# Gteam1-EE/srsRAN_Project_23.5

Hardware: AMD Instinct MI355X
Metric: LDPC info-bits/sec + OFDM slots/sec, 100 MHz n78 273-PRB grid (higher is better)
Workload: dtype int8; 1 GPU; 273-PRB 30kHz PUSCH, 256QAM R=948/1024, 1 layer, 38 CB/slot BG1 Z=384, TBS 319784; per slot, time-domain samples to transport block: OFDM demod (4096-pt, 1 port) + DM-RS channel estimate + equalise/soft-demap/descramble + rate-dematch + LDPC decode (6 it, early_stop=0) + TB assembly/CRC24A; slots synthesised by the transmit chain + AWGN; parallelism=slots sharded across GPUs, no data-path collective

## Files before the change

srsran_project_23.5_amd/csrc/ldpc_decode_pk.hip:

```cpp
#include "miphy_internal.h"
#include "rdm_device.h"
#include "ldpc_frame_device.h"
#include <algorithm>
#include <cstdlib>

namespace {

__device__ __forceinline__ bool block_crc_is_zero(const int8_t* soft, const miphy_graph_tables* __restrict__ tab, int zi, int order, int L,
                                                  uint32_t* red, int tid, int nt)
{
  return block_xor(crc_zmask_partial(soft, tab, zi, order, L, tid, nt), red, tid, nt) == 0;
}

__device__ __forceinline__ uint32_t block_crc(const int8_t* soft, const miphy_graph_tables* __restrict__ tab, int crc_id, uint32_t poly,
                                              uint32_t order, int K, int L, uint32_t* red, int tid, int nt)
{
  return block_xor(crc_div_partial(soft, tab, crc_id, poly, order, K, L, tid, nt), red, tid, nt);
}

#ifdef LDPC_PK_PROFILE
__device__ unsigned long long g_ldpc_prof[2048 * 8];
#define PROF_T(var) const unsigned long long var = __builtin_amdgcn_s_memtime()
#define PROF_ADD(slot, a, b) prof_acc[slot] += (unsigned long long)((b) - (a))
#define PROF_COUNT()                                              \
  do {                                                            \
    if (tid == 0 && blockIdx.x < 2048) {                          \
      for (int q = 0; q < 7; ++q)                                 \
        g_ldpc_prof[blockIdx.x * 8 + q] += prof_acc[q];           \
      g_ldpc_prof[blockIdx.x * 8 + 7] += 1;                       \
    }                                                             \
    for (int q = 0; q < 7; ++q)                                   \
      prof_acc[q] = 0;                                            \
  } while (0)
#else
#define PROF_T(var)
#define PROF_ADD(slot, a, b)
#define PROF_COUNT()
#endif

#define LDPC_PK_MIN_WAVES_PLAIN 4
#ifndef LDPC_PK_MIN_WAVES_SPLIT
#define LDPC_PK_MIN_WAVES_SPLIT 3
#endif
#ifndef LDPC_PK_MIN_WAVES_FUSED
#define LDPC_PK_MIN_WAVES_FUSED 3
#endif
struct raw_in16 {
  uint32_t a0, a1, a2, a3, e;
};
__device__ __forceinline__ raw_in16 load_in16_raw(const int8_t* __restrict__ in, int mb, int v)
{
  const uint32_t* p4 = reinterpret_cast<const uint32_t*>(in - mb) + 4 * v;
  const rdm_u4    a  = *reinterpret_cast<const rdm_u4*>(p4);
  raw_in16        r;
  r.a0 = a.x, r.a1 = a.y, r.a2 = a.z, r.a3 = a.w;
  r.e  = (mb != 0) ? p4[4] : 0u;
  return r;
}
__device__ __forceinline__ uint4 shift_in16(const raw_in16& r, int mb)
{
  if (mb == 0)
    return make_uint4(r.a0, r.a1, r.a2, r.a3);
  return make_uint4(__builtin_amdgcn_alignbyte(r.a1, r.a0, mb), __builtin_amdgcn_alignbyte(r.a2, r.a1, mb), __builtin_amdgcn_alignbyte(r.a3, r.a2, mb),
                    __builtin_amdgcn_alignbyte(r.e, r.a3, mb));
}
constexpr int PK_PRE = 3;

__device__ __forceinline__ int pk_in16_vectors(int mb, int E)
{
  return (mb == 0) ? (E >> 4) : ((E >= 4) ? ((E - 4) >> 4) : 0);
}
__device__ __forceinline__ void pk_prefetch(raw_in16 (&pre)[PK_PRE], uint32_t c, uint32_t n, const miphy_ldpc_rdm_desc* __restrict__ rdm,
                                            const int8_t* __restrict__ rm_in_base, const uint32_t* __restrict__ cb_order, int tid, int nt)
{
#pragma unroll
  for (int k = 0; k < PK_PRE; ++k)
    pre[k] = raw_in16{0, 0, 0, 0, 0};
  if (c < n) {
    const miphy_ldpc_rdm_desc r  = load_words(rdm + (cb_order ? cb_order[c] : c));
    const int8_t*             in = rm_in_base + r.in_offset;
    const int                 mb = (int)(((uintptr_t)in) & 3), nq = pk_in16_vectors(mb, (int)r.E);
#pragma unroll
    for (int k = 0; k < PK_PRE; ++k) {
      pre[k] = raw_in16{0, 0, 0, 0, 0};
      if (tid + k * nt < nq)
        pre[k] = load_in16_raw(in, mb, tid + k * nt);
    }
  }
}

typedef __attribute__((address_space(1))) const int8_t* global_ci8;
__device__ __attribute__((noinline)) void pk_fused_load(int8_t* __restrict__ soft, global_ci8 in_global, int E, int F, int mod, int Z, int bgK, int soft_bytes,
                                                        raw_in16 p0, raw_in16 p1, raw_in16 p2, int tid, int nt)
{
  static_assert(PK_PRE == 3, "three prefetched vectors are passed by value");
  const int8_t* __restrict__ in = (const int8_t*)in_global;
    int stid = tid;
    asm volatile("" : "+v"(stid));
    const int                 mb  = (int)(((uintptr_t)in) & 3);
    const int                 nq  = pk_in16_vectors(mb, E);
    int8_t*                   img = soft + 2 * Z;
    rm_geom                   g;
    g.r0 = 0, g.f1 = (bgK - 2) * Z, g.f0 = g.f1 - F, g.F = F, g.E = E, g.mod = mod, g.Kq = E / mod;
    image_access ia;
    ia.jbase = 0;
    {
      uint4* z4 = reinterpret_cast<uint4*>(soft);
      for (int k = stid; k < (2 * Z) >> 4; k += nt)
        z4[k] = make_uint4(0, 0, 0, 0);
      for (int k = g.f0 + stid; k < g.f1; k += nt)
        img[k] = 127;
      for (int k = 2 * Z + E + F + stid; k < soft_bytes; k += nt)
        soft[k] = 0;
    }
    switch (mod) {
#define PK_STAGE(MOD)                                                                         \
  case MOD:                                                                                   \
    _Pragma("unroll") for (int k = 0; k < PK_PRE; ++k) if (stid + k * nt < nq)                 \
        stage_vector<MOD>(ia, img, g, F, stid + k * nt, shift_in16(k == 0 ? p0 : (k == 1 ? p1 : p2), mb));               \
    for (int v = stid + PK_PRE * nt; v < nq; v += nt)                                          \
      stage_vector<MOD>(ia, img, g, F, v, load_in16(in, mb, v));                              \
    break;
      PK_STAGE(8)
      PK_STAGE(6)
      PK_STAGE(4)
      PK_STAGE(2)
      default:
        PK_STAGE(1)
#undef PK_STAGE
    }
    for (int k = (nq << 4) + stid; k < E; k += nt) {
      const int p = k / (int)mod, q = k - p * (int)mod;
      const int r = q * g.Kq + p;
      img[r + ((r >= g.f0) ? F : 0)] = in[k];
    }
    __syncthreads();
}

__device__ __forceinline__ int pk_fused_image_out(const int8_t* __restrict__ soft, int8_t* __restrict__ llr_img, int Z, int bgi, int in_len, int tid, int nt)
{
  typedef uint32_t u32x4 __attribute__((ext_vector_type(4)));
  int          last = 0;
  u32x4*       dst  = reinterpret_cast<u32x4*>(llr_img);
  const uint4* src  = reinterpret_cast<const uint4*>(soft + 2 * Z);
  const int    nimg = in_len >> 4, nall = ((miphy_bg_N_short(bgi) * Z) >> 4);
  asm volatile("" : "+v"(tid));
  for (int q = tid; q < nimg; q += nt) {
    const uint4 v = src[q];
    const u32x4 o = {v.x, v.y, v.z, v.w};
    __builtin_nontemporal_store(o, dst + q);
    last = last_nonzero_behind(v, q, last);
  }
  const u32x4 zero = {0, 0, 0, 0};
  for (int q = nimg + tid; q < nall; q += nt)
    __builtin_nontemporal_store(zero, dst + q);
  return last;
}

constexpr int PK_ATAB_DEGREE = MIPHY_LDPC_ADR_TABLE_DEGREE, PK_ATAB_QUADS = (PK_ATAB_DEGREE + 3) / 4;
template <bool FUSED, bool GMSG, int PARTS = 1, bool ATAB = false, bool RSKIP = false>
__global__ void __launch_bounds__(192 * PARTS, PARTS > 1 ? LDPC_PK_MIN_WAVES_SPLIT : (FUSED ? LDPC_PK_MIN_WAVES_FUSED : LDPC_PK_MIN_WAVES_PLAIN))
ldpc_decode_pk_kernel(const miphy_ldpc_dec_desc* __restrict__ descs,
                      const miphy_graph_tables* __restrict__ tab,
                      const int8_t* __restrict__ llr_base,
                      uint8_t* __restrict__ out_base,
                      int32_t* __restrict__ iters_out,
                      int max_nodes,
                      const uint32_t* __restrict__ harq_slot,
                      uint8_t* __restrict__ harq_crc_ok,
                      uint32_t n,
                      uint32_t* __restrict__ queue,
                      const miphy_ldpc_rdm_desc* __restrict__ rdm,
                      const int8_t* __restrict__ rm_in_base,
                      uint32_t* __restrict__ gmsg,
                      int gmsg_pairs,
                      int lds_pairs,
                      const uint32_t* __restrict__ cb_order,
                      const pk_adr_quad* const* __restrict__ adr_by_z)
{
  extern __shared__ __attribute__((aligned(16))) unsigned char smem[];
  const int tid = threadIdx.x;
  const int nt  = blockDim.x;
  constexpr bool SPLIT = PARTS > 1;
  static_assert(PARTS == 1 || PARTS == 2 || PARTS == 4, "parts of the latency form");
  static_assert(!(SPLIT && GMSG), "the latency form keeps its messages in LDS");
  static_assert(!ATAB || (FUSED && !GMSG && !SPLIT), "address tables: the throughput form that dematches, messages in LDS");
  static_assert(!(RSKIP && (SPLIT || GMSG)), "visits are left out by the throughput forms with their messages in LDS");
  const int nth  = nt / PARTS;
  const int part = SPLIT ? __builtin_amdgcn_readfirstlane((tid >= nth) + (PARTS > 2 ? (tid >= 2 * nth) + (tid >= 3 * nth) : 0)) : 0;
  const int lr   = tid - part * nth;
  raw_in16  pre[PK_PRE];
  if (FUSED)
    pk_prefetch(pre, blockIdx.x, n, rdm, rm_in_base, cb_order, tid, nt);
#ifdef LDPC_PK_PROFILE
  unsigned long long prof_acc[7] = {};
#endif
  for (uint32_t q = blockIdx.x; q < n;) {
  __builtin_amdgcn_s_setprio(LDPC_PK_SETPRIO_OUT);
  PROF_T(p_start);
  const uint32_t cb = cb_order ? cb_order[q] : q;
  const miphy_ldpc_dec_desc dsc = load_words(descs + cb);
  const int                 Z   = dsc.Z;
  const int                 H   = (Z + 1) >> 1;
  const int                 bgi = (dsc.bg == 1) ? 0 : 1;
  const int                 bgK = miphy_bg_K(bgi);
  const int                 bgM = miphy_bg_M(bgi);
  const int                 K   = bgK * Z;
  const int                 zp  = tab->z_pos[Z];

  int8_t*   soft       = reinterpret_cast<int8_t*>(smem);
  const int lay_alloc  = miphy_ldpc_layers(bgi, max_nodes);
  const int soft_bytes = miphy_ldpc_soft_bytes(bgi, lay_alloc, Z);
  const int pairs_all  = tab->pair_start[bgi][lay_alloc];
  const int pairs_lds  = GMSG ? lds_pairs : pairs_all;
  uint32_t* c2v_lane   = reinterpret_cast<uint32_t*>(smem + soft_bytes) + (lr >> 6) * (pairs_lds * 64) + (lr & 63);
  uint32_t* c2v_glob   = GMSG ? gmsg + ((size_t)blockIdx.x * (nt >> 6) + (tid >> 6)) * ((size_t)gmsg_pairs * 64) + (tid & 63) - 64 * (size_t)pairs_lds : nullptr;
  uint32_t* red        = reinterpret_cast<uint32_t*>(smem + soft_bytes) + (nth >> 6) * (pairs_lds * 64);
  uint32_t* xch = red + 16 + lr;

  __syncthreads();
  if (tid == 0) {
    const uint32_t ticket = atomicAdd(queue, 1u);
    if (ticket == n - 1u)
      *queue = 0u;
    red[15] = gridDim.x + ticket;
  }
  if (!FUSED && harq_crc_ok && harq_crc_ok[harq_slot[cb]]) {
    if (tid == 0)
      iters_out[cb] = -1;
    __syncthreads();
    q = red[15];
    continue;
  }
  const int8_t* llr    = llr_base + dsc.llr_offset;
  uint8_t*      out    = out_base + dsc.out_offset;
  const int     in_len = (int)dsc.in_len;

  if (tid < 15)
    red[tid] = 0;
  int last = 0;
  auto prefetch = [&](uint32_t c) { pk_prefetch(pre, c, n, rdm, rm_in_base, cb_order, tid, nt); };
  pk_adr_quad    anx[ATAB ? PK_ATAB_QUADS : 1];
  pk_adr_row     atab    = pk_adr_row();
  const uint32_t astride = 16u * (uint32_t)nt, alayer = PK_ATAB_QUADS * astride;
  if (ATAB) {
    const int zq = __builtin_amdgcn_readfirstlane(Z >> 4), bytes = __builtin_amdgcn_readfirstlane(lay_alloc * (int)alayer);
    atab.rsrc    = __builtin_amdgcn_make_buffer_rsrc(const_cast<pk_adr_quad*>(adr_by_z[zq]), 0, bytes, 0x00020000);
    atab.soff = alayer;
    pk_table_request<PK_ATAB_DEGREE>(anx, atab, 16u * (uint32_t)tid, astride);
  }
  if (FUSED) {
    const miphy_ldpc_rdm_desc rd = load_words(rdm + cb);
    pk_fused_load(soft, (global_ci8)(rm_in_base + rd.in_offset), (int)rd.E, (int)dsc.nof_filler_bits, (int)rd.mod, Z, bgK, soft_bytes, pre[0], pre[1], pre[2], tid, nt);
    last = pk_fused_image_out(soft, const_cast<int8_t*>(llr), Z, bgi, in_len, tid, nt);
  } else {
    last = cb_plain_load(soft, llr, in_len, Z, soft_bytes, tid, nt);
  }
  atomicMax(reinterpret_cast<int*>(&red[0]), last);
  __syncthreads();
  last = (int)red[0];

  const bool use_crc = dsc.crc_poly != MIPHY_CRC_NONE;
  if (last == 0) {
    if (!use_crc) {
      store_all_ones(out, K, tid, nt);
    }
    if (tid == 0) {
      iters_out[cb] = 0;
      if (FUSED && harq_crc_ok)
        harq_crc_ok[harq_slot[cb]] = 0;
    }
    if (FUSED)
      prefetch(red[15]);
    q = red[15];
    continue;
  }
  const int nof_layers = cb_nof_layers(last, Z, bgi);

  const uint32_t* edges_g   = tab->edge_sb[bgi][zp];
  uint32_t lay_info = 0;
  {
    const int ml = tid & 63;
    if (ml < bgM) {
      const uint32_t e0 = tab->row_start[bgi][ml];
      lay_info          = e0 | (((uint32_t)tab->row_start[bgi][ml + 1] - e0) << 10) | ((uint32_t)tab->pair_start[bgi][ml] << 16);
    }
  }
  uint32_t        poly = 0, order = 0;
  int             L = 0;
  if (use_crc) {
    poly  = tab->crc_poly[dsc.crc_poly];
    order = tab->crc_order[dsc.crc_poly];
    L     = K - dsc.nof_filler_bits;
  }
  const bool final_only = use_crc && (dsc.flags & 1u);
  const int zi = (use_crc && L <= 32 * MIPHY_CRC_ZMASK_WORDS) ? miphy_crc_zmask_index(dsc.crc_poly) : -1;

  int       result_iters = 0;
  const int max_iter     = dsc.max_iter;
  PROF_T(p_loaded);
  PROF_ADD(0, p_start, p_loaded);
  int Zv = Z, Hv = (lr + H < Z) ? H : 0;
#ifndef LDPC_PK_SCALAR_WRAP
  asm volatile("" : "+v"(Zv), "+v"(Hv));
#endif
  __builtin_amdgcn_s_setprio(LDPC_PK_SETPRIO1);
  part_edges<PARTS> pe;
  if (SPLIT)
    load_part_edges<PARTS>(pe, edges_g, (uint32_t)__builtin_amdgcn_readlane((int)lay_info, 1), part);
  [[maybe_unused]] uint64_t sat_layers = 0;
  for (int it = 0; it < max_iter; ++it) {
    for (int m = (it == 0) ? 1 : 0; m < nof_layers; ++m) {
      const uint32_t  li    = (uint32_t)__builtin_amdgcn_readlane((int)lay_info, m);
      const int       e0    = (int)(li & 0x3ffu);
      const int       d     = (int)((li >> 10) & 0x3fu);
      const uint32_t* edges = edges_g + 2 * e0;
      PROF_T(p_l0);
      if constexpr (SPLIT) {
        part_edges<PARTS> pn;
        const uint32_t    lin  = (uint32_t)__builtin_amdgcn_readlane((int)lay_info, (m + 1 < nof_layers) ? m + 1 : 0);
        auto              next = [&]() { load_part_edges<PARTS>(pn, edges_g, lin, part); };
        const pk_exchange<decltype(next)> x = {xch, part, nth, lr < H, next};
        uint32_t* cl = c2v_lane + 64 * (li >> 16);
        if (it == 0 || (it == 1 && m == 0))
          update_rows_pk_split<true, PARTS>(pe, soft, cl, lr, Hv, Zv, x);
        else
          update_rows_pk_split<false, PARTS>(pe, soft, cl, lr, Hv, Zv, x);
        pe = pn;
      } else if constexpr (!RSKIP) {
        if (ATAB) {
          if (tid < H)
            update_rows_pk_visit_tab<PK_ATAB_DEGREE>(it, m, soft, c2v_lane + 64 * (li >> 16),
                                                     pk_adr_table{anx, {atab.rsrc, (uint32_t)__builtin_amdgcn_readfirstlane((m + 1 < nof_layers) ? m + 1 : 0) * alayer},
                                                                  16u * (uint32_t)tid, astride});
        } else if (tid < H) {
          if (GMSG && (int)(li >> 16) >= pairs_lds) {
            update_rows_pk_visit<FUSED>(it, m, d, soft, c2v_glob + 64 * (li >> 16), pk_adr_computed{edges, tid, Hv, Zv, 0});
          } else {
            update_rows_pk_visit<FUSED>(it, m, d, soft, c2v_lane + 64 * (li >> 16), pk_adr_computed{edges, tid, Hv, Zv, 0});
          }
        }
      } else if (!((sat_layers >> m) & 1u)) {
        bool all_inf = false;
        if (ATAB) {
          const uint64_t live = ~sat_layers & (((uint64_t)1 << nof_layers) - 1u), above = live & ~(((uint64_t)2 << m) - 1u);
          const int      mn   = __builtin_amdgcn_readfirstlane(above ? __builtin_ctzll(above) : __builtin_ctzll(live));
          if (tid < H)
            all_inf = update_rows_pk_visit_tab<PK_ATAB_DEGREE, true>(it, m, soft, c2v_lane + 64 * (li >> 16),
                                                                     pk_adr_table{anx, {atab.rsrc, (uint32_t)mn * alayer}, 16u * (uint32_t)tid, astride});
        } else if (tid < H) {
          if (GMSG && (int)(li >> 16) >= pairs_lds) {
            all_inf = update_rows_pk_visit<FUSED, true>(it, m, d, soft, c2v_glob + 64 * (li >> 16), pk_adr_computed{edges, tid, Hv, Zv, 0});
          } else {
            all_inf = update_rows_pk_visit<FUSED, true>(it, m, d, soft, c2v_lane + 64 * (li >> 16), pk_adr_computed{edges, tid, Hv, Zv, 0});
          }
        }
        if (__builtin_amdgcn_ballot_w64(tid < H && !all_inf) == 0)
          sat_layers |= (uint64_t)1 << m;
      }
      PROF_T(p_l1);
      __syncthreads();
      PROF_T(p_l2);
      PROF_ADD(1, p_l0, p_l1);
      PROF_ADD(2, p_l1, p_l2);
    }
    if (use_crc && !final_only) {
      if (zi >= 0 ? block_crc_is_zero(soft, tab, zi, (int)order, L, red, tid, nt) : block_crc(soft, tab, dsc.crc_poly, poly, order, K, L, red, tid, nt) == 0) {
        result_iters = it + 1;
        break;
      }
    }
  }
  PROF_T(p_dec);
  __builtin_amdgcn_s_setprio(LDPC_PK_SETPRIO_OUT);
  if (FUSED) {
    prefetch(red[15]);
  }
  if (final_only)
    result_iters = (zi >= 0 ? block_crc_is_zero(soft, tab, zi, (int)order, L, red, tid, nt) : block_crc(soft, tab, dsc.crc_poly, poly, order, K, L, red, tid, nt) == 0)
                       ? max_iter
                       : 0;
  PROF_T(p_crc);
  PROF_ADD(3, p_dec, p_crc);

  store_hard_words(soft, out, K, tid, nt);
  if (tid == 0) {
    iters_out[cb] = result_iters;
    if (harq_crc_ok && (FUSED || result_iters > 0))
      harq_crc_ok[harq_slot[cb]] = result_iters > 0;
  }
  PROF_T(p_end);
  PROF_ADD(4, p_crc, p_end);
  PROF_ADD(5, p_start, p_end);
  PROF_COUNT();
  q = red[15];
  }
}

struct pk_instance_key {
  bool fused, gmsg;
  int  parts;
  bool atab, row_skip;
  constexpr bool operator==(const pk_instance_key& o) const { return fused == o.fused && gmsg == o.gmsg && parts == o.parts && atab == o.atab && row_skip == o.row_skip; }
};
typedef decltype(&ldpc_decode_pk_kernel<false, false>) pk_kernel_fn;
struct pk_instance {
  pk_instance_key key;
  pk_kernel_fn    kernel;
};
template <bool FUSED, bool GMSG, int PARTS = 1, bool ATAB = false, bool RSKIP = false>
constexpr pk_instance pk_instance_of()
{
  return {{FUSED, GMSG, PARTS, ATAB, RSKIP}, ldpc_decode_pk_kernel<FUSED, GMSG, PARTS, ATAB, RSKIP>};
}
constexpr pk_instance pk_instances[] = {
    pk_instance_of<false, false>(),        pk_instance_of<false, true>(),         pk_instance_of<true, false>(),         pk_instance_of<true, true>(),
    pk_instance_of<false, false, 2>(),     pk_instance_of<true, false, 2>(),      pk_instance_of<false, false, 4>(),     pk_instance_of<true, false, 4>(),
    pk_instance_of<true, false, 1, true>(), pk_instance_of<false, false, 1, false, true>(), pk_instance_of<true, false, 1, false, true>(),
    pk_instance_of<true, false, 1, true, true>(),
};

}

#ifdef LDPC_PK_PROFILE
extern "C" int miphy_debug_ldpc_profile(unsigned long long out[8], int reset)
{
  static unsigned long long h[2048 * 8];
  if (hipMemcpyFromSymbol(h, HIP_SYMBOL(g_ldpc_prof), sizeof(h)) != hipSuccess)
    return -1;
  for (int q = 0; q < 8; ++q) {
    out[q] = 0;
    for (int b = 0; b < 2048; ++b)
      out[q] += h[b * 8 + q];
  }
  if (reset) {
    for (auto& v : h)
      v = 0;
    if (hipMemcpyToSymbol(HIP_SYMBOL(g_ldpc_prof), h, sizeof(h)) != hipSuccess)
      return -1;
  }
  return 0;
}
#endif

#ifdef LDPC_PK_PROFILE2
extern "C" int miphy_debug_ldpc_profile2(unsigned long long out[8], int reset)
{
  if (hipMemcpyFromSymbol(out, HIP_SYMBOL(g_ldpc_prof2), 8 * sizeof(unsigned long long)) != hipSuccess)
    return -1;
  if (reset) {
    unsigned long long z[8] = {};
    if (hipMemcpyToSymbol(HIP_SYMBOL(g_ldpc_prof2), z, sizeof(z)) != hipSuccess)
      return -1;
  }
  return 0;
}
#endif

int miphy_ldpc_pk_waves_per_cu(bool fused, int parts)
{
#ifdef LDPC_PK_REPORT_WAVES_FUSED
  if (fused && parts <= 1)
    return 4 * LDPC_PK_REPORT_WAVES_FUSED;
#endif
  return 4 * (parts > 1 ? LDPC_PK_MIN_WAVES_SPLIT : (fused ? LDPC_PK_MIN_WAVES_FUSED : LDPC_PK_MIN_WAVES_PLAIN));
}

size_t miphy_ldpc_pk_lds_bytes(int bgi, int lay, size_t Zt, int pairs_all, int parts)
{
  const size_t waves = ((Zt + 1) / 2 + 63) / 64;
  return (size_t)miphy_ldpc_soft_bytes(bgi, lay, (int)Zt) + waves * (size_t)pairs_all * 256 + 64 + (parts > 1 ? (size_t)parts * 3 * 64 * waves * 4 : 0);
}

int miphy_ldpc_pk_per_cu(size_t lds, int waves, bool fused, int parts)
{
  return std::max(1, std::min((int)((size_t)160 * 1024 / lds), miphy_ldpc_pk_waves_per_cu(fused, parts) / waves));
}

uint32_t miphy_ldpc_pk_grid(const miphy_ctx* ctx, uint32_t n, int threads, size_t lds, bool fused, int parts)
{
  return std::min<uint32_t>(n, (uint32_t)(ctx->num_cus * miphy_ldpc_pk_per_cu(lds, threads / 64, fused, parts)));
}

int miphy_ldpc_pk_launch(miphy_ctx* ctx, const miphy_ldpc_launch& L, const miphy_ldpc_dec_desc* d_descs, const uint32_t* d_order, const int8_t* llr,
                         uint8_t* out_bits, int32_t* iters, const uint32_t* harq_slot, uint8_t* harq_crc_ok, const miphy_ldpc_rdm_desc* d_rdm,
                         const int8_t* rm_in, void* gmsg, hipStream_t s)
{
  const bool fused = (L.used & MIPHY_LDPC_KERNEL_FUSED) != 0, gm = L.gmsg_pairs > 0;
  MIPHY_REQUIRE(L.threads <= 1024, "ldpc_decode: workgroup of %d threads", L.threads);
  const pk_instance_key want = {fused, gm, L.parts, L.adr_by_z != nullptr, L.row_skip};
  pk_kernel_fn          kern = nullptr;
  for (const pk_instance& i : pk_instances)
    if (i.key == want)
      kern = i.kernel;
  MIPHY_REQUIRE(kern, "ldpc_decode: no packed kernel instance {fused %d, global messages %d, parts %d, address table %d, row skip %d}", want.fused, want.gmsg, want.parts,
                want.atab, want.row_skip);
  if (L.lds > 48 * 1024) {
    MIPHY_HIP_CHECK(hipFuncSetAttribute((const void*)kern, hipFuncAttributeMaxDynamicSharedMemorySize, (int)L.lds));
  }
  uint32_t* queue = nullptr;
  int       rc    = miphy_next_queue_counter(ctx, &queue);
  if (rc)
    return rc;
  hipLaunchKernelGGL(kern, dim3(L.grid), dim3(L.threads), L.lds, s, d_descs, ctx->d_tables, llr, out_bits, iters, L.nodes, harq_slot, harq_crc_ok, L.c.count, queue, d_rdm,
                     rm_in, (uint32_t*)gmsg, L.gmsg_pairs, gm ? L.lds_pairs : 0, d_order, (const pk_adr_quad* const*)L.adr_by_z);
  MIPHY_HIP_CHECK(hipGetLastError());
  return MIPHY_OK;
}
```

srsran_project_23.5_amd/csrc/ldpc_pk_device.h:

```cpp
#pragma once
#include "miphy_internal.h"
#include <type_traits>

namespace {

typedef short s16x2 __attribute__((ext_vector_type(2)));

__device__ __forceinline__ s16x2 as_s2(uint32_t x)
{
  return __builtin_bit_cast(s16x2, x);
}
__device__ __forceinline__ uint32_t as_u(s16x2 x)
{
  return __builtin_bit_cast(uint32_t, x);
}
__device__ __forceinline__ s16x2 splat(int c)
{
  return s16x2{(short)c, (short)c};
}
__device__ __forceinline__ s16x2 pk_min(s16x2 a, s16x2 b)
{
  return __builtin_elementwise_min(a, b);
}
__device__ __forceinline__ s16x2 pk_max(s16x2 a, s16x2 b)
// ... 324 lines not shown
    }
  }
  __builtin_amdgcn_s_setprio(LDPC_PK_SETPRIO2);
  if constexpr (ATAB)
    pk_table_request<D>(adr.q, adr.next, adr.voff, adr.stride);
  const uint32_t sA = ((uint32_t)(uint16_t)mag.x * 52428u) >> 16, sB = ((uint32_t)(uint16_t)mag.y * 52428u) >> 16;
  const s16x2    pm = pk_ashr15(as_s2(spx));
  const s16x2    c  = as_s2((sA | (sB << 16)) ^ as_u(pm)) - pm;
  const uint32_t r  = as_u(c);
  c2v[0] = ZE ? c2v_pack(splat(0), c) : c2v_pack(c, splat(0));
#pragma unroll
  for (int jj = 1; jj < (D + 1) / 2; ++jj)
    c2v[64 * jj] = 0u;
  pk_soft_bit<ATAB>(soft, adrA[ZE]) = (int8_t)r;
  pk_soft_bit<ATAB>(soft, adrB[ZE]) = (int8_t)(r >> 16);
  __builtin_amdgcn_s_setprio(LDPC_PK_SETPRIO1);
}

template <typename MID>
__device__ __forceinline__ void update_rows_pk_none(pk_exchange<MID> x)
{
  uint32_t* xw = x.xch + 3 * x.part * x.xs;
  xw[0] = as_u(splat(LLR_MAX)), xw[x.xs] = as_u(splat(LLR_MAX)), xw[2 * x.xs] = 0u;
  __syncthreads();
  x.mid();
}

template <int PARTS>
struct part_edges {
  static constexpr int EMAX = PARTS == 4 ? 6 : 10;
  uint32_t             w[2 * EMAX];
  int                  da;
  int                  p0;
};

template <int PARTS>
__device__ __forceinline__ void load_part_edges(part_edges<PARTS>& pe, const uint32_t* __restrict__ edges_g, uint32_t li, int part)
{
  const int d = (int)((li >> 10) & 0x3fu), P = (d + 1) >> 1;
  const int p0 = (P * part) / PARTS, p1 = (P * (part + 1)) / PARTS;
  pe.p0 = p0, pe.da = min(2 * p1, d) - 2 * p0;
  const uint32_t* e = edges_g + 2 * ((int)(li & 0x3ffu) + 2 * p0);
#pragma unroll
  for (int k = 0; k < 2 * part_edges<PARTS>::EMAX; ++k)
    pe.w[k] = e[k];
}

template <bool FIRST, int PARTS, typename MID>
__device__ __forceinline__ void update_rows_pk_split(const part_edges<PARTS>& pe, int8_t* soft, uint32_t* c2v, int l, int H, int Z, pk_exchange<MID> x)
{
  const pk_adr_computed adr = {pe.w, l, H, Z, 0};
  c2v += 64 * pe.p0;
  switch (pe.da) {
#define PK_SPLIT_CASE(N)                                                                            \
  case N:                                                                                           \
    if (N <= part_edges<PARTS>::EMAX)                                                               \
      update_rows_pk<(N <= part_edges<PARTS>::EMAX ? N : 1), FIRST, PARTS, false>(soft, c2v, adr, x); \
    break;
    PK_SPLIT_CASE(10)
    PK_SPLIT_CASE(9)
    PK_SPLIT_CASE(6)
    PK_SPLIT_CASE(5)
    PK_SPLIT_CASE(4)
    PK_SPLIT_CASE(3)
    PK_SPLIT_CASE(2)
    PK_SPLIT_CASE(1)
    default:
      update_rows_pk_none(x);
      break;
#undef PK_SPLIT_CASE
  }
}

template <bool FIRST, bool FOLD, bool DETECT = false>
__device__ __forceinline__ bool update_rows_pk_any(int d, int8_t* soft, uint32_t* c2v, pk_adr_computed adr)
{
  switch (d) {
#define PK_ANY_CASE(N) \
  case N:              \
    return update_rows_pk<N, FIRST, 1, FOLD, DETECT>(soft, c2v, adr);
    PK_ANY_CASE(19)
    PK_ANY_CASE(10)
    PK_ANY_CASE(9)
    PK_ANY_CASE(8)
    PK_ANY_CASE(7)
    PK_ANY_CASE(6)
    PK_ANY_CASE(5)
    PK_ANY_CASE(4)
#undef PK_ANY_CASE
    default:
      return update_rows_pk<3, FIRST, 1, FOLD, DETECT>(soft, c2v, adr);
  }
}

template <bool FOLD>
__device__ __forceinline__ void update_rows_pk_zero_any(int m, int d, int8_t* soft, uint32_t* c2v, pk_adr_computed adr)
{
  if (m == 1) {
    if (d == 19)
      update_rows_pk_zero<19, 0, FOLD>(soft, c2v, adr);
    else
      update_rows_pk_zero<10, 0, FOLD>(soft, c2v, adr);
  } else {
    if (d == 19)
      update_rows_pk_zero<19, 1, FOLD>(soft, c2v, adr);
    else
      update_rows_pk_zero<8, 1, FOLD>(soft, c2v, adr);
  }
}

template <bool FOLD, bool DETECT = false>
__device__ __forceinline__ bool update_rows_pk_visit(int it, int m, int d, int8_t* soft, uint32_t* c2v, pk_adr_computed adr)
{
  bool r = false;
  if (it == 0 && (m == 1 || m == 2))
    update_rows_pk_zero_any<FOLD>(m, d, soft, c2v, adr);
  else if (it == 0 || (it == 1 && m == 0))
    r = update_rows_pk_any<true, FOLD, DETECT>(d, soft, c2v, adr);
  else
    r = update_rows_pk_any<false, FOLD, DETECT>(d, soft, c2v, adr);
  return r;
}

template <int D, bool DETECT = false>
__device__ __forceinline__ bool update_rows_pk_visit_tab(int it, int m, int8_t* soft, uint32_t* c2v, pk_adr_table adr)
{
  if (it == 0 && m == 1) {
    update_rows_pk_zero<D, 0, true>(soft, c2v, adr);
    return false;
  }
  if (it == 0 && m == 2) {
    update_rows_pk_zero<D, 1, true>(soft, c2v, adr);
    return false;
  }
  if (it == 0 || (it == 1 && m == 0))
    return update_rows_pk<D, true, 1, true, DETECT>(soft, c2v, adr);
  return update_rows_pk<D, false, 1, true, DETECT>(soft, c2v, adr);
}

__device__ __forceinline__ uint32_t gf2_mulmod(uint32_t a, uint32_t b, uint32_t poly, uint32_t order)
{
  uint32_t       r   = 0;
  const uint32_t top = 1u << order;
  for (int k = (int)order - 1; k >= 0; --k) {
    r <<= 1;
    r ^= (r & top) ? poly : 0u;
    r ^= ((b >> k) & 1u) ? a : 0u;
  }
  return r;
}

__device__ __forceinline__ uint32_t hard_word(const int8_t* soft, int t, int K)
{
  const uint32_t* p = reinterpret_cast<const uint32_t*>(soft) + 8 * t;
  uint32_t        w = 0;
#pragma unroll
  for (int q = 0; q < 8; ++q) {
    const uint32_t x = p[q];
#pragma unroll
    for (int b = 0; b < 4; ++b) {
      const int v = (int8_t)(x >> (8 * b));
      w |= (uint32_t)(v <= 0) << (31 - (4 * q + b));
    }
  }
  const int rem = K - 32 * t;
  if (rem < 32)
    w &= (rem <= 0) ? 0u : (0xffffffffu << (32 - rem));
  return w;
}

__device__ __forceinline__ uint32_t hard_flags(const int8_t* soft, int t)
{
  const uint4* p  = reinterpret_cast<const uint4*>(soft) + 2 * t;
  const uint4  lo = p[0], hi = p[1];
  const uint32_t x[8] = {lo.x, lo.y, lo.z, lo.w, hi.x, hi.y, hi.z, hi.w};
  uint32_t       w    = 0;
#pragma unroll
  for (int q = 7; q >= 0; --q) {
    const uint32_t nz  = (x[q] & 0x7f7f7f7fu) + 0x7f7f7f7fu;
    const uint32_t le0 = (x[q] | ~nz) & 0x80808080u;
    w                  = (w << 1) | (le0 >> 7);
  }
  return w;
}

__device__ __forceinline__ uint32_t crc_zmask_partial(const int8_t* soft, const miphy_graph_tables* __restrict__ tab, int zi, int order, int L, int first,
                                                      int stride)
{
  const int nw = (L + 31) >> 5;
  uint32_t  acc[24];
#pragma unroll
  for (int k = 0; k < 24; ++k)
    acc[k] = 0;
  for (int t = first; t < nw; t += stride) {
    uint32_t  w   = hard_flags(soft, t);
    const int rem = L - 32 * t;
    if (rem < 32) {
      uint32_t valid = 0;
      for (int q = 0; q < 8; ++q) {
        const int      nb = min(4, max(0, rem - 4 * q));
        const uint32_t lo = (nb >= 4) ? 0xffffffffu : ((1u << (8 * nb)) - 1u);
        valid |= (0x01010101u & lo) << q;
      }
      w &= valid;
    }
    const uint4* m = reinterpret_cast<const uint4*>(tab->crc_zmask[zi][nw - 1 - t]);
#pragma unroll
    for (int g = 0; g < 6; ++g) {
      const uint4 mk = m[g];
      acc[4 * g + 0] += __builtin_popcount(w & mk.x);
      acc[4 * g + 1] += __builtin_popcount(w & mk.y);
      acc[4 * g + 2] += __builtin_popcount(w & mk.z);
      acc[4 * g + 3] += __builtin_popcount(w & mk.w);
    }
  }
  uint32_t par = 0;
#pragma unroll
  for (int k = 0; k < 24; ++k)
    par |= (acc[k] & 1u) << k;
  return par & ((1u << order) - 1u);
}

__device__ __forceinline__ uint32_t crc_div_partial(const int8_t* soft, const miphy_graph_tables* __restrict__ tab, int crc_id, uint32_t poly, uint32_t order,
                                                    int K, int L, int first, int stride)
{
  const int      nfull = L >> 5, rbits = L & 31, nwords = (L + 31) >> 5;
  const uint32_t top   = 1u << order;
  uint32_t       part  = 0;
  for (int t = first; t < nwords; t += stride) {
    const uint32_t w   = hard_word(soft, t, K);
    const int      len = min(32, L - 32 * t);
    uint32_t       reg = 0;
    for (int b = 0; b < len; ++b) {
      reg = (reg << 1) ^ (((w >> (31 - b)) & 1u) << order);
      reg ^= (reg & top) ? poly : 0u;
    }
    reg &= top - 1u;
    if (t < nfull) {
      reg = gf2_mulmod(reg, tab->crc_pow32[crc_id][nfull - 1 - t], poly, order);
      for (int b = 0; b < rbits; ++b) {
        reg <<= 1;
        reg ^= (reg & top) ? poly : 0u;
      }
    }
    part ^= reg;
  }
  return part;
}

__device__ __forceinline__ uint32_t block_xor(uint32_t part, uint32_t* red, int tid, int nt)
{
#pragma unroll
  for (int off = 32; off >= 1; off >>= 1)
    part ^= __shfl_xor(part, off);
  if ((tid & 63) == 0)
    red[2 + (tid >> 6)] = part;
  __syncthreads();
  uint32_t crc = 0;
  for (int w = 0; w < (nt >> 6); ++w)
    crc ^= red[2 + w];
  __syncthreads();
  return crc;
}

__device__ __forceinline__ void store_hard_words(const int8_t* soft, uint8_t* out, int K, int first, int stride, uint32_t base = 0)
{
  const bool out_aligned = ((uintptr_t)out & 3u) == 0;
  const int  kwords      = (K + 31) >> 5;
  for (int t = first; t < kwords; t += stride) {
    const uint32_t w      = hard_word(soft + base, t, K);
    const int      nbytes = min(4, (K - 32 * t + 7) / 8);
    if (nbytes == 4 && out_aligned) {
      reinterpret_cast<uint32_t*>(out)[t] = __builtin_bswap32(w);
    } else {
      for (int q = 0; q < nbytes; ++q)
        out[4 * t + q] = (uint8_t)(w >> (24 - 8 * q));
    }
  }
}

}
```

srsran_project_23.5_amd/csrc/miphy_ctx.hip:

```cpp
#include "miphy_internal.h"
#include "miphy_ext.h"
#include "tables/nr_ldpc_tables.h"
#include <algorithm>
#include <cstdarg>
#include <cstdlib>
#include <cstring>
#include <new>

static thread_local char g_err[512] = "";

void miphy_set_error(const char* fmt, ...)
{
  va_list ap;
  va_start(ap, fmt);
  vsnprintf(g_err, sizeof(g_err), fmt, ap);
  va_end(ap);
}

extern "C" const char* miphy_last_error(void)
{
  return g_err;
}

extern "C" int miphy_version(void)
{
  return MIPHY_VERSION;
}

static int lifting_set(int Z)
{
  static const int A[8] = {2, 3, 5, 7, 9, 11, 13, 15};
  for (int i = 7; i >= 0; --i) {
    if (Z % A[i])
      continue;
    int q = Z / A[i];
    if ((q & (q - 1)) == 0)
      return i;
  }
  return -1;
}

static uint32_t gf2_mulmod(uint32_t a, uint32_t b, uint32_t poly, unsigned order)
{
  uint32_t r = 0, top = 1u << order;
  for (int i = (int)order - 1; i >= 0; --i) {
    r <<= 1;
    if (r & top)
      r ^= poly;
    if ((b >> i) & 1u)
      r ^= a;
  }
  return r;
}

static bool first_layers_as_decoded(const uint16_t* row_start, const uint8_t* col, int d1, int d2)
{
  bool has0 = false, has1 = false;
  for (int e = row_start[0]; e < row_start[1]; ++e)
    has0 |= col[e] == 0, has1 |= col[e] == 1;
  bool ok = has0 && has1 && row_start[2] - row_start[1] == d1 && row_start[3] - row_start[2] == d2;
  ok &= col[row_start[1]] == 0 && col[row_start[2]] == 0 && col[row_start[2] + 1] == 1;
  for (int e = row_start[1] + 1; e < row_start[2]; ++e)
    ok &= col[e] > 1;
  for (int e = row_start[2] + 2; e < row_start[3]; ++e)
    ok &= col[e] > 1;
  return ok;
}

static void build_tables(miphy_graph_tables* t)
{
  memset(t, 0, sizeof(*t));
  for (int z = 0; z <= MIPHY_MAX_Z; ++z) {
    t->z_pos[z] = 0xffff;
    t->i_ls[z]  = 0xff;
  }
  for (int p = 0; p < MIPHY_NOF_Z; ++p) {
    int Z        = NR_LDPC_LIFTING_SIZES[p];
    t->z_pos[Z]  = (uint16_t)p;
    int ils      = lifting_set(Z);
    t->i_ls[Z]   = (uint8_t)ils;
    for (int e = 0; e < NR_LDPC_BG1_NOF_EDGES; ++e)
      t->edge[0][p][e] = (uint32_t)(NR_LDPC_BG1_COL[e] * Z) | ((uint32_t)(NR_LDPC_BG1_SHIFT[ils][e] % Z) << 16);
    for (int e = 0; e < NR_LDPC_BG2_NOF_EDGES; ++e)
      t->edge[1][p][e] = (uint32_t)(NR_LDPC_BG2_COL[e] * Z) | ((uint32_t)(NR_LDPC_BG2_SHIFT[ils][e] % Z) << 16);
  }
  for (int b = 0; b < 2; ++b)
    for (int p = 0; p < MIPHY_NOF_Z; ++p)
      for (int e = 0; e < (b ? NR_LDPC_BG2_NOF_EDGES : NR_LDPC_BG1_NOF_EDGES); ++e) {
        t->edge_sb[b][p][2 * e]     = t->edge[b][p][e] >> 16;
        t->edge_sb[b][p][2 * e + 1] = t->edge[b][p][e] & 0xffffu;
      }
  for (int m = 0; m <= NR_LDPC_BG1_M; ++m)
    t->row_start[0][m] = NR_LDPC_BG1_ROW_START[m];
  for (int m = 0; m <= NR_LDPC_BG2_M; ++m)
    t->row_start[1][m] = NR_LDPC_BG2_ROW_START[m];
  for (int b = 0; b < 2; ++b) {
    t->pair_start[b][0] = 0;
    for (int m = 0; m < (b ? NR_LDPC_BG2_M : NR_LDPC_BG1_M); ++m)
      t->pair_start[b][m + 1] = (uint16_t)(t->pair_start[b][m] + (t->row_start[b][m + 1] - t->row_start[b][m] + 1) / 2);
  }
  static const uint32_t POLY[5]  = {0x1864CFB, 0x1800063, 0x1B2B117, 0x11021, 0xE21};
  static const uint32_t ORDER[5] = {24, 24, 24, 16, 11};
  for (int p = 0; p < 5; ++p) {
    t->crc_poly[p]  = POLY[p];
    t->crc_order[p] = ORDER[p];
    uint32_t x32 = 1, top = 1u << ORDER[p];
    for (int i = 0; i < 32; ++i) {
      x32 <<= 1;
      if (x32 & top)
        x32 ^= POLY[p];
    }
    uint32_t v = 1;
    for (int k = 0; k < 320; ++k) {
      t->crc_pow32[p][k] = v;
      v                  = gf2_mulmod(v, x32, POLY[p], ORDER[p]);
    }
    {
      const uint32_t x8192 = gf2_mulmod(t->crc_pow32[p][255], x32, POLY[p], ORDER[p]);
      uint32_t       h     = 1;
      for (int k = 0; k < 256; ++k) {
        t->crc_pow32_hi[p][k] = h;
        h                     = gf2_mulmod(h, x8192, POLY[p], ORDER[p]);
      }
    }
    v = x32;
    for (int b = 0; b < 24; ++b) {
      t->crc_pow2[p][b] = v;
      v                 = gf2_mulmod(v, v, POLY[p], ORDER[p]);
    }
    const int zi = miphy_crc_zmask_index(p);
    if (zi >= 0) {
      uint32_t c = 1;
      for (unsigned i = 0; i < ORDER[p]; ++i) {
        c <<= 1;
        if (c & top)
          c ^= POLY[p];
      }
      for (int u = 0; u < MIPHY_CRC_ZMASK_WORDS; ++u)
        for (int jl = 0; jl < 32; ++jl) {
          const int i_local = 31 - jl, q = i_local >> 2, b = i_local & 3;
          for (unsigned k = 0; k < ORDER[p]; ++k)
            if ((c >> k) & 1u) {
              t->crc_zmask[zi][u][k] |= 1u << (q + 8 * b);
              if (p == 0)
                t->crc_zmask_packed24a[u][k] |= 1u << (8 * (i_local >> 3) + 7 - (i_local & 7));
            }
          c <<= 1;
          if (c & top)
            c ^= POLY[p];
        }
    }
  }
}

extern "C" int miphy_ldpc_address_table(int bg, int Z, int layers, uint32_t* out)
{
  MIPHY_REQUIRE(bg == 1 || bg == 2, "miphy_ldpc_address_table: invalid base graph %d", bg);
  MIPHY_REQUIRE(Z >= 2 && Z <= MIPHY_MAX_Z && lifting_set(Z) >= 0, "miphy_ldpc_address_table: invalid lifting size %d", Z);
  MIPHY_REQUIRE(layers >= 1 && layers <= (bg == 1 ? NR_LDPC_BG1_M : NR_LDPC_BG2_M), "miphy_ldpc_address_table: invalid number of layers %d", layers);
  const uint16_t* row_start = bg == 1 ? NR_LDPC_BG1_ROW_START : NR_LDPC_BG2_ROW_START;
  const uint8_t*  col       = bg == 1 ? NR_LDPC_BG1_COL : NR_LDPC_BG2_COL;
  const int       ils = lifting_set(Z), H = (Z + 1) / 2, lanes = 64 * ((H + 63) / 64);
  size_t          quad = 0;
  for (int m = 0; m < layers; ++m) {
    const int e0 = row_start[m], d = row_start[m + 1] - e0, nq = (d + 3) / 4;
    if (out) {
      for (int j = 0; j < 4 * nq; ++j) {
        const int      e  = e0 + std::min(j, d - 1);
        const uint32_t sh = (uint32_t)((bg == 1 ? NR_LDPC_BG1_SHIFT[ils][e] : NR_LDPC_BG2_SHIFT[ils][e]) % Z), co = (uint32_t)col[e] * Z;
        for (int l = 0; l < lanes; ++l) {
          uint32_t w = 0;
          if (l < H) {
            const uint16_t Hv = (l + H < Z) ? (uint16_t)H : 0;
            const uint16_t tA = (uint16_t)(l + sh), tB = (uint16_t)(l + Hv + sh);
            const uint16_t rA = std::min<uint16_t>(tA, (uint16_t)(tA - Z)), rB = std::min<uint16_t>(tB, (uint16_t)(tB - Z));
            w                 = ((uint32_t)rA + co) | (((uint32_t)rB + co) << 16);
          }
          out[((quad + j / 4) * lanes + l) * 4 + j % 4] = w;
        }
      }
    }
    quad += nq;
  }
  return (int)(quad * lanes * 4);
}

int miphy_ldpc_address_tables(miphy_ctx* ctx, int bgi, int lay, int min_Z, int max_Z, const void** out)
{
  constexpr int    NZ = MIPHY_MAX_Z / 16 + 1;
  ldpc_adr_tables& T  = ctx->ext->ldpc_adr[{bgi, lay}];
  if (!T.d_ptr) {
    const void* none[NZ] = {};
    if (int rc = miphy_keep_device_copy(ctx, none, sizeof(none), (void**)&T.d_ptr))
      return rc;
  }
  for (int Z = min_Z; Z <= max_Z; ++Z) {
    if (ctx->h_tables->z_pos[Z] == 0xffff || T.h_ptr[Z / 16])
      continue;
    MIPHY_REQUIRE(Z % 16 == 0, "ldpc address tables: lifting size %d has no table index of its own", Z);
    const int words = miphy_ldpc_address_table(bgi + 1, Z, lay, nullptr);
    if (words < 0)
      return words;
    std::vector<uint32_t> h((size_t)words);
    (void)miphy_ldpc_address_table(bgi + 1, Z, lay, h.data());
    void* d = nullptr;
    if (int rc = miphy_keep_device_copy(ctx, h.data(), h.size() * 4, &d))
      return rc;
    MIPHY_HIP_CHECK(hipMemcpy(T.d_ptr + Z / 16, &d, sizeof(void*), hipMemcpyHostToDevice));
    T.h_ptr[Z / 16] = d;
  }
  *out = T.d_ptr;
  return MIPHY_OK;
}

extern "C" int miphy_create(int device, miphy_ctx** out)
{
  if (!out) {
    miphy_set_error("miphy_create: null out pointer");
    return MIPHY_EINVAL;
  }
  *out = nullptr;
  MIPHY_REQUIRE(first_layers_as_decoded(NR_LDPC_BG1_ROW_START, NR_LDPC_BG1_COL, 19, 19) && first_layers_as_decoded(NR_LDPC_BG2_ROW_START, NR_LDPC_BG2_COL, 10, 8),
                "miphy_create: layers 0-2 of the LDPC base graph tables are not what the decoders' first iteration relies on");
  MIPHY_HIP_CHECK(hipSetDevice(device));
  miphy_ctx* c = new (std::nothrow) miphy_ctx();
  if (!c)
    return MIPHY_ENOMEM;
  c->device   = device;
  c->num_cus  = 256;
  (void)hipDeviceGetAttribute(&c->num_cus, hipDeviceAttributeMultiprocessorCount, device);
  c->ext      = new miphy_ctx_ext();
  c->h_tables = (miphy_graph_tables*)malloc(sizeof(miphy_graph_tables));
  build_tables(c->h_tables);
  MIPHY_HIP_CHECK(hipMalloc((void**)&c->d_tables, sizeof(miphy_graph_tables)));
  MIPHY_HIP_CHECK(hipMemcpy(c->d_tables, c->h_tables, sizeof(miphy_graph_tables), hipMemcpyHostToDevice));
  c->desc_staging_bytes = 8u << 20;
  c->staging_head       = 0;
  MIPHY_HIP_CHECK(hipMalloc(&c->d_desc_staging, c->desc_staging_bytes));
  MIPHY_HIP_CHECK(hipHostMalloc(&c->h_desc_staging, c->desc_staging_bytes, hipHostMallocDefault));
  MIPHY_HIP_CHECK(hipMalloc((void**)&c->d_queue, MIPHY_NOF_QUEUE_COUNTERS * sizeof(uint32_t)));
  MIPHY_HIP_CHECK(hipMemset(c->d_queue, 0, MIPHY_NOF_QUEUE_COUNTERS * sizeof(uint32_t)));
  c->queue_next = 0;
  *out = c;
  return MIPHY_OK;
}

extern "C" void miphy_destroy(miphy_ctx* c)
{
  if (!c)
    return;
  (void)hipSetDevice(c->device);
  (void)hipFree(c->d_tables);
  for (void* p : c->ext->to_free)
    (void)hipFree(p);
  delete c->ext;
  for (int k = 0; k < MIPHY_NOF_SIDE_STREAMS; ++k) {
    if (c->side_stream[k])
      (void)hipStreamDestroy((hipStream_t)c->side_stream[k]);
    if (c->ev_join[k])
      (void)hipEventDestroy((hipEvent_t)c->ev_join[k]);
  }
  if (c->ev_fork)
    (void)hipEventDestroy((hipEvent_t)c->ev_fork);
  (void)hipFree(c->d_desc_staging);
  (void)hipFree(c->d_queue);
  for (void* w : c->d_work)
    (void)hipFree(w);
  (void)hipHostFree(c->h_desc_staging);
  free(c->h_tables);
  delete c;
}

int miphy_side_streams(miphy_ctx* ctx)
{
  if (ctx->ev_fork)
    return MIPHY_OK;
  for (int k = 0; k < MIPHY_NOF_SIDE_STREAMS; ++k) {
    hipStream_t st = nullptr;
    hipEvent_t  e  = nullptr;
    MIPHY_HIP_CHECK(hipStreamCreateWithFlags(&st, hipStreamNonBlocking));
    MIPHY_HIP_CHECK(hipEventCreateWithFlags(&e, hipEventDisableTiming));
    ctx->side_stream[k] = st, ctx->ev_join[k] = e;
  }
  hipEvent_t f = nullptr;
  MIPHY_HIP_CHECK(hipEventCreateWithFlags(&f, hipEventDisableTiming));
  ctx->ev_fork = f;
  return MIPHY_OK;
}

int miphy_next_queue_counter(miphy_ctx* ctx, uint32_t** out)
{
  *out = ctx->d_queue + (ctx->queue_next++ % MIPHY_NOF_QUEUE_COUNTERS);
  return MIPHY_OK;
}

static int staging_take(miphy_ctx* ctx, size_t bytes, hipStream_t s, size_t* off)
// ... 145 lines not shown
```

Before: 112.8 billion info_bits/s.

## Reuse CRC hard words for output, vectorize hard decision, scan last-nonzero backward

```diff
diff --git a/srsran_project_23.5_amd/csrc/ldpc_decode_pk.hip b/srsran_project_23.5_amd/csrc/ldpc_decode_pk.hip
--- a/srsran_project_23.5_amd/csrc/ldpc_decode_pk.hip
+++ b/srsran_project_23.5_amd/csrc/ldpc_decode_pk.hip
@@ -6,10 +6,11 @@
 
 namespace {
 
-__device__ __forceinline__ bool block_crc_is_zero(const int8_t* soft, const miphy_graph_tables* __restrict__ tab, int zi, int order, int L,
-                                                  uint32_t* red, int tid, int nt)
-{
-  return block_xor(crc_zmask_partial(soft, tab, zi, order, L, tid, nt), red, tid, nt) == 0;
+template <bool KEEP>
+__device__ __forceinline__ bool block_crc_is_zero(const int8_t* soft, const miphy_graph_tables* __restrict__ tab, int zi, int order, int L, int K,
+                                                  uint32_t* kept, uint32_t* red, int tid, int nt)
+{
+  return block_xor(crc_zmask_partial<KEEP>(soft, tab, zi, order, L, tid, nt, K, kept), red, tid, nt) == 0;
 }
 
 __device__ __forceinline__ uint32_t block_crc(const int8_t* soft, const miphy_graph_tables* __restrict__ tab, int crc_id, uint32_t poly,
@@ -137,10 +138,9 @@
     __syncthreads();
 }
 
-__device__ __forceinline__ int pk_fused_image_out(const int8_t* __restrict__ soft, int8_t* __restrict__ llr_img, int Z, int bgi, int in_len, int tid, int nt)
+__device__ __forceinline__ int pk_fused_image_out(const int8_t* __restrict__ soft, int8_t* __restrict__ llr_img, int Z, int bgi, int in_len, int end, int tid, int nt)
 {
   typedef uint32_t u32x4 __attribute__((ext_vector_type(4)));
-  int          last = 0;
   u32x4*       dst  = reinterpret_cast<u32x4*>(llr_img);
   const uint4* src  = reinterpret_cast<const uint4*>(soft + 2 * Z);
   const int    nimg = in_len >> 4, nall = ((miphy_bg_N_short(bgi) * Z) >> 4);
@@ -149,11 +149,18 @@
     const uint4 v = src[q];
     const u32x4 o = {v.x, v.y, v.z, v.w};
     __builtin_nontemporal_store(o, dst + q);
-    last = last_nonzero_behind(v, q, last);
   }
   const u32x4 zero = {0, 0, 0, 0};
   for (int q = nimg + tid; q < nall; q += nt)
     __builtin_nontemporal_store(zero, dst + q);
+  int last = 0;
+  for (int hi = __builtin_amdgcn_readfirstlane((min(end, in_len) - 1) >> 4); hi >= 0; hi -= 64) {
+    const int q = hi - (tid & 63);
+    if (q >= 0)
+      last = last_nonzero_behind(src[q], q, 0);
+    if (__builtin_amdgcn_ballot_w64(last != 0))
+      break;
+  }
   return last;
 }
 
@@ -182,6 +189,7 @@
   const int tid = threadIdx.x;
   const int nt  = blockDim.x;
   constexpr bool SPLIT = PARTS > 1;
+  constexpr bool KEEPW = FUSED && !SPLIT;
   static_assert(PARTS == 1 || PARTS == 2 || PARTS == 4, "parts of the latency form");
   static_assert(!(SPLIT && GMSG), "the latency form keeps its messages in LDS");
   static_assert(!ATAB || (FUSED && !GMSG && !SPLIT), "address tables: the throughput form that dematches, messages in LDS");
@@ -252,7 +260,7 @@
   if (FUSED) {
     const miphy_ldpc_rdm_desc rd = load_words(rdm + cb);
     pk_fused_load(soft, (global_ci8)(rm_in_base + rd.in_offset), (int)rd.E, (int)dsc.nof_filler_bits, (int)rd.mod, Z, bgK, soft_bytes, pre[0], pre[1], pre[2], tid, nt);
-    last = pk_fused_image_out(soft, const_cast<int8_t*>(llr), Z, bgi, in_len, tid, nt);
+    last = pk_fused_image_out(soft, const_cast<int8_t*>(llr), Z, bgi, in_len, (int)rd.E + (int)dsc.nof_filler_bits, tid, nt);
   } else {
     last = cb_plain_load(soft, llr, in_len, Z, soft_bytes, tid, nt);
   }
@@ -298,6 +306,7 @@
 
   int       result_iters = 0;
   const int max_iter     = dsc.max_iter;
+  uint32_t  kept[2]      = {0, 0};
   PROF_T(p_loaded);
   PROF_ADD(0, p_start, p_loaded);
   int Zv = Z, Hv = (lr + H < Z) ? H : 0;
@@ -365,7 +374,7 @@
       PROF_ADD(2, p_l1, p_l2);
     }
     if (use_crc && !final_only) {
-      if (zi >= 0 ? block_crc_is_zero(soft, tab, zi, (int)order, L, red, tid, nt) : block_crc(soft, tab, dsc.crc_poly, poly, order, K, L, red, tid, nt) == 0) {
+      if (zi >= 0 ? block_crc_is_zero<KEEPW>(soft, tab, zi, (int)order, L, K, kept, red, tid, nt) : block_crc(soft, tab, dsc.crc_poly, poly, order, K, L, red, tid, nt) == 0) {
         result_iters = it + 1;
         break;
       }
@@ -377,13 +386,16 @@
     prefetch(red[15]);
   }
   if (final_only)
-    result_iters = (zi >= 0 ? block_crc_is_zero(soft, tab, zi, (int)order, L, red, tid, nt) : block_crc(soft, tab, dsc.crc_poly, poly, order, K, L, red, tid, nt) == 0)
+    result_iters = (zi >= 0 ? block_crc_is_zero<KEEPW>(soft, tab, zi, (int)order, L, K, kept, red, tid, nt) : block_crc(soft, tab, dsc.crc_poly, poly, order, K, L, red, tid, nt) == 0)
                        ? max_iter
                        : 0;
   PROF_T(p_crc);
   PROF_ADD(3, p_dec, p_crc);
 
-  store_hard_words(soft, out, K, tid, nt);
+  if (KEEPW && zi >= 0 && (final_only || max_iter > 0))
+    store_kept_words(soft, out, K, tid, nt, kept);
+  else
+    store_hard_words(soft, out, K, tid, nt);
   if (tid == 0) {
     iters_out[cb] = result_iters;
     if (harq_crc_ok && (FUSED || result_iters > 0))
diff --git a/srsran_project_23.5_amd/csrc/ldpc_pk_device.h b/srsran_project_23.5_amd/csrc/ldpc_pk_device.h
--- a/srsran_project_23.5_amd/csrc/ldpc_pk_device.h
+++ b/srsran_project_23.5_amd/csrc/ldpc_pk_device.h
@@ -500,57 +500,53 @@
 
 __device__ __forceinline__ uint32_t hard_word(const int8_t* soft, int t, int K)
 {
-  const uint32_t* p = reinterpret_cast<const uint32_t*>(soft) + 8 * t;
-  uint32_t        w = 0;
-#pragma unroll
-  for (int q = 0; q < 8; ++q) {
-    const uint32_t x = p[q];
-#pragma unroll
-    for (int b = 0; b < 4; ++b) {
-      const int v = (int8_t)(x >> (8 * b));
-      w |= (uint32_t)(v <= 0) << (31 - (4 * q + b));
-    }
-  }
+  const uint4*   p  = reinterpret_cast<const uint4*>(soft) + 2 * t;
+  const uint4    lo = p[0], hi = p[1];
+  const uint32_t x[8] = {lo.x, lo.y, lo.z, lo.w, hi.x, hi.y, hi.z, hi.w};
+  uint32_t       h[2];
+#pragma unroll
+  for (int k = 0; k < 2; ++k) {
+    uint32_t acc = 0;
+#pragma unroll
+    for (int q = 4 * k; q < 4 * k + 4; ++q) {
+      const uint32_t xq  = x[q ^ 1];
+      const uint32_t nz  = (xq & 0x7f7f7f7fu) + 0x7f7f7f7fu;
+      const uint32_t pos = ~xq & nz & 0x80808080u;
+      if (q == 4 * k + 2)
+        acc <<= 8;
+      acc = __builtin_amdgcn_udot4(pos, (q & 1) ? 0x10204080u : 0x01020408u, acc, false);
+    }
+    h[k] = acc;
+  }
+  uint32_t  w   = ~((h[0] << 9) | (h[1] >> 7));
   const int rem = K - 32 * t;
   if (rem < 32)
     w &= (rem <= 0) ? 0u : (0xffffffffu << (32 - rem));
   return w;
 }
 
-__device__ __forceinline__ uint32_t hard_flags(const int8_t* soft, int t)
-{
-  const uint4* p  = reinterpret_cast<const uint4*>(soft) + 2 * t;
-  const uint4  lo = p[0], hi = p[1];
-  const uint32_t x[8] = {lo.x, lo.y, lo.z, lo.w, hi.x, hi.y, hi.z, hi.w};
-  uint32_t       w    = 0;
-#pragma unroll
-  for (int q = 7; q >= 0; --q) {
-    const uint32_t nz  = (x[q] & 0x7f7f7f7fu) + 0x7f7f7f7fu;
-    const uint32_t le0 = (x[q] | ~nz) & 0x80808080u;
-    w                  = (w << 1) | (le0 >> 7);
-  }
-  return w;
-}
-
+template <bool KEEP = false>
 __device__ __forceinline__ uint32_t crc_zmask_partial(const int8_t* soft, const miphy_graph_tables* __restrict__ tab, int zi, int order, int L, int first,
-                                                      int stride)
-{
-  const int nw = (L + 31) >> 5;
+                                                      int stride, int K = 0, uint32_t* kept = nullptr)
+{
+  const int nw = (L + 31) >> 5, nk = KEEP ? (K + 31) >> 5 : nw;
   uint32_t  acc[24];
 #pragma unroll
   for (int k = 0; k < 24; ++k)
     acc[k] = 0;
-  for (int t = first; t < nw; t += stride) {
-    uint32_t  w   = hard_flags(soft, t);
-    const int rem = L - 32 * t;
-    if (rem < 32) {
-      uint32_t valid = 0;
-      for (int q = 0; q < 8; ++q) {
-        const int      nb = min(4, max(0, rem - 4 * q));
-        const uint32_t lo = (nb >= 4) ? 0xffffffffu : ((1u << (8 * nb)) - 1u);
-        valid |= (0x01010101u & lo) << q;
-      }
-      w &= valid;
+  [[maybe_unused]] uint32_t k0 = 0, k1 = 0;
+  [[maybe_unused]] int      i  = 0;
+  for (int t = first; t < nk; t += stride) {
+    uint32_t w = hard_word(soft, t, KEEP ? K : L);
+    if constexpr (KEEP) {
+      k0 = (i == 0) ? w : k0;
+      k1 = (i == 1) ? w : k1;
+      ++i;
+      if (t >= nw)
+        continue;
+      const int rem = L - 32 * t;
+      if (rem < 32)
+        w &= 0xffffffffu << (32 - rem);
     }
     const uint4* m = reinterpret_cast<const uint4*>(tab->crc_zmask[zi][nw - 1 - t]);
 #pragma unroll
@@ -562,11 +558,13 @@
       acc[4 * g + 3] += __builtin_popcount(w & mk.w);
     }
   }
+  if constexpr (KEEP)
+    kept[0] = k0, kept[1] = k1;
   uint32_t par = 0;
 #pragma unroll
   for (int k = 0; k < 24; ++k)
-    par |= (acc[k] & 1u) << k;
-  return par & ((1u << order) - 1u);
+    par = __builtin_amdgcn_alignbit(acc[k], par, 1);
+  return (par >> 8) & ((1u << order) - 1u);
 }
 
 __device__ __forceinline__ uint32_t crc_div_partial(const int8_t* soft, const miphy_graph_tables* __restrict__ tab, int crc_id, uint32_t poly, uint32_t order,
@@ -611,20 +609,35 @@
   return crc;
 }
 
+__device__ __forceinline__ void store_hard_word(uint8_t* out, bool out_aligned, uint32_t w, int t, int K)
+{
+  const int nbytes = min(4, (K - 32 * t + 7) / 8);
+  if (nbytes == 4 && out_aligned) {
+    reinterpret_cast<uint32_t*>(out)[t] = __builtin_bswap32(w);
+  } else {
+    for (int q = 0; q < nbytes; ++q)
+      out[4 * t + q] = (uint8_t)(w >> (24 - 8 * q));
+  }
+}
+
 __device__ __forceinline__ void store_hard_words(const int8_t* soft, uint8_t* out, int K, int first, int stride, uint32_t base = 0)
 {
   const bool out_aligned = ((uintptr_t)out & 3u) == 0;
   const int  kwords      = (K + 31) >> 5;
-  for (int t = first; t < kwords; t += stride) {
-    const uint32_t w      = hard_word(soft + base, t, K);
-    const int      nbytes = min(4, (K - 32 * t + 7) / 8);
-    if (nbytes == 4 && out_aligned) {
-      reinterpret_cast<uint32_t*>(out)[t] = __builtin_bswap32(w);
-    } else {
-      for (int q = 0; q < nbytes; ++q)
-        out[4 * t + q] = (uint8_t)(w >> (24 - 8 * q));
-    }
-  }
-}
-
-}
+  for (int t = first; t < kwords; t += stride)
+    store_hard_word(out, out_aligned, hard_word(soft + base, t, K), t, K);
+}
+
+__device__ __forceinline__ void store_kept_words(const int8_t* soft, uint8_t* out, int K, int first, int stride, const uint32_t* kept)
+{
+  const bool out_aligned = ((uintptr_t)out & 3u) == 0;
+  const int  kwords      = (K + 31) >> 5;
+  if (first < kwords)
+    store_hard_word(out, out_aligned, kept[0], first, K);
+  if (first + stride < kwords)
+    store_hard_word(out, out_aligned, kept[1], first + stride, K);
+  for (int t = first + 2 * stride; t < kwords; t += stride)
+    store_hard_word(out, out_aligned, hard_word(soft, t, K), t, K);
+}
+
+}
diff --git a/srsran_project_23.5_amd/csrc/miphy_ctx.hip b/srsran_project_23.5_amd/csrc/miphy_ctx.hip
--- a/srsran_project_23.5_amd/csrc/miphy_ctx.hip
+++ b/srsran_project_23.5_amd/csrc/miphy_ctx.hip
@@ -138,10 +138,10 @@
       }
       for (int u = 0; u < MIPHY_CRC_ZMASK_WORDS; ++u)
         for (int jl = 0; jl < 32; ++jl) {
-          const int i_local = 31 - jl, q = i_local >> 2, b = i_local & 3;
+          const int i_local = 31 - jl;
           for (unsigned k = 0; k < ORDER[p]; ++k)
             if ((c >> k) & 1u) {
-              t->crc_zmask[zi][u][k] |= 1u << (q + 8 * b);
+              t->crc_zmask[zi][u][k] |= 1u << jl;
               if (p == 0)
                 t->crc_zmask_packed24a[u][k] |= 1u << (8 * (i_local >> 3) + 7 - (i_local & 7));
             }
```

Measured after the change: 122.0 billion info_bits/s (median of 6 runs). +8.1%, better.
